# iden3/snarkjs

Measured on NVIDIA H100. Metric: groth16_proofs_per_sec, higher is better.
Workload: dtype u32x8 (256-bit modular integers, 32-bit limbs)

## Files before the change

### snarkjs_b200/csrc/ec.cuh

```cuda
#pragma once
#include "fp.cuh"

namespace sb {

template <class P> struct Fp2 {
    typedef Fp<P> B;
    static constexpr bool HAS_MUL2 = false;
    B a, b;
    SB_HD static Fp2 one() { Fp2 r; r.a = B::one(); r.b = B::zero(); return r; }
    SB_HD static Fp2 inv(const Fp2& x) {
        B t = B::inv_binary(B::add(B::sqr(x.a), B::sqr(x.b)));
        Fp2 r; r.a = B::mul(x.a, t); r.b = B::neg(B::mul(x.b, t)); return r;
    }
    SB_HD static Fp2 zero() { Fp2 r; r.a = B::zero(); r.b = B::zero(); return r; }
    SB_HD bool is_zero() const { return a.is_zero() & b.is_zero(); }
    SB_HD bool operator==(const Fp2& o) const { return (a == o.a) & (b == o.b); }
    SB_HD static Fp2 add(const Fp2& x, const Fp2& y) { Fp2 r; r.a = B::add(x.a, y.a); r.b = B::add(x.b, y.b); return r; }
    SB_HD static Fp2 sub(const Fp2& x, const Fp2& y) { Fp2 r; r.a = B::sub(x.a, y.a); r.b = B::sub(x.b, y.b); return r; }
    SB_HD static Fp2 dbl(const Fp2& x) { Fp2 r; r.a = B::dbl(x.a); r.b = B::dbl(x.b); return r; }
    SB_HD static Fp2 neg(const Fp2& x) { Fp2 r; r.a = B::neg(x.a); r.b = B::neg(x.b); return r; }
    SB_HD static Fp2 cneg(const Fp2& x, bool f) { Fp2 r; r.a = B::cneg(x.a, f); r.b = B::cneg(x.b, f); return r; }
    SB_HD_NOINLINE static Fp2 mul(const Fp2& x, const Fp2& y) { return mul_i(x, y); }
    SB_HD_NOINLINE static Fp2 sqr(const Fp2& x) { return sqr_i(x); }
    SB_HD static Fp2 mul_i(const Fp2& x, const Fp2& y) {
#if defined(__CUDA_ARCH__) && defined(SB_FP2_LAZY)
        return mul_lazy(x, y);
#endif
        if constexpr (B::HAS_MUL2) {
            Fp2 r; r.a = B::mul2(x.a, y.a, x.b, B::neg(y.b)); r.b = B::mul2(x.a, y.b, x.b, y.a); return r;
        } else {
            B A = B::mul(x.a, y.a), Bb = B::mul(x.b, y.b);
            B C = B::mul(B::add(x.a, x.b), B::add(y.a, y.b));
            Fp2 r; r.a = B::sub(A, Bb); r.b = B::sub(B::sub(C, A), Bb); return r;
        }
    }
    SB_HD static Fp2 mul_lazy(const Fp2& x, const Fp2& y) {
        constexpr int N = B::N;
        uint32_t v0[2 * N], v1[2 * N], v2[2 * N], sa[N], sb[N];
        B::mul_wide(x.a.v, y.a.v, v0);
        B::mul_wide(x.b.v, y.b.v, v1);
        B::add_noreduce(x.a, x.b, sa); B::add_noreduce(y.a, y.b, sb);
        B::mul_wide(sa, sb, v2);
        B::wide_sub(v2, v0); B::wide_sub(v2, v1);
        uint32_t bw = B::wide_sub(v0, v1);
        B::wide_add_p_high(v0, bw);
        Fp2 r; r.a = B::redc_wide(v0); r.b = B::redc_wide(v2); return r;
    }
    SB_HD static Fp2 sqr_i(const Fp2& x) {
        B AB = B::mul(x.a, x.b);
        Fp2 r; r.a = B::mul(B::add(x.a, x.b), B::sub(x.a, x.b)); r.b = B::dbl(AB); return r;
    }
};

template <class F> struct Affine {
    F x, y;
    SB_HD bool is_inf() const { return x.is_zero() & y.is_zero(); }
};

template <class F> struct XYZZ {
    F x, y, zz, zzz;
    SB_HD static XYZZ inf() { XYZZ r; r.x = F::zero(); r.y = F::zero(); r.zz = F::zero(); r.zzz = F::zero(); return r; }
    SB_HD bool is_inf() const { return zz.is_zero(); }

    SB_HD_NOINLINE static XYZZ dbl_affine(const F& px, const F& py, const F& one) {
        XYZZ r;
        if (py.is_zero()) return inf();
        F U = F::dbl(py), V = F::sqr(U), W = F::mul(U, V), S = F::mul(px, V);
        F M = F::sqr(px); M = F::add(F::dbl(M), M);
        r.x = F::sub(F::sqr(M), F::dbl(S));
        r.y = F::sub(F::mul(M, F::sub(S, r.x)), F::mul(W, py));
        r.zz = V; r.zzz = W;
        (void)one;
        return r;
    }
    SB_HD_NOINLINE static XYZZ dbl(const XYZZ& p) {
        if (p.is_inf() || p.y.is_zero()) return inf();
        XYZZ r;
        F U = F::dbl(p.y), V = F::sqr(U), W = F::mul(U, V), S = F::mul(p.x, V);
        F M = F::sqr(p.x); M = F::add(F::dbl(M), M);
        r.x = F::sub(F::sqr(M), F::dbl(S));
        r.y = F::sub(F::mul(M, F::sub(S, r.x)), F::mul(W, p.y));
        r.zz = F::mul(V, p.zz); r.zzz = F::mul(W, p.zzz);
        return r;
    }
    SB_HD void add_affine(const F& qx, const F& qy, const F& one) {
        if (is_inf()) { x = qx; y = qy; zz = one; zzz = one; return; }
        F U2 = F::mul_i(qx, zz), S2 = F::mul_i(qy, zzz);
        F Pp = F::sub(U2, x), R = F::sub(S2, y);
        if (Pp.is_zero()) {
            if (R.is_zero()) *this = dbl_affine(qx, qy, one);
            else *this = inf();
            return;
        }
        F PP = F::sqr_i(Pp), PPP = F::mul_i(Pp, PP), Q = F::mul_i(x, PP);
        F X3 = F::sub(F::sub(F::sqr_i(R), PPP), F::dbl(Q));
        F Y3;
        if constexpr (F::HAS_MUL2) Y3 = F::mul2_i(R, F::sub(Q, X3), F::neg(y), PPP);
        else Y3 = F::sub(F::mul_i(R, F::sub(Q, X3)), F::mul_i(y, PPP));
        x = X3; y = Y3; zz = F::mul_i(zz, PP); zzz = F::mul_i(zzz, PPP);
    }
    SB_HD void add_i(const XYZZ& q) {
        if (q.is_inf()) return;
        if (is_inf()) { *this = q; return; }
        F U1 = F::mul_i(x, q.zz), S1 = F::mul_i(y, q.zzz);
        F ZZ = F::mul_i(zz, q.zz), ZZZ = F::mul_i(zzz, q.zzz);
        F Pp = F::sub(F::mul_i(q.x, zz), U1), R = F::sub(F::mul_i(q.y, zzz), S1);
        if (Pp.is_zero()) {
            if (R.is_zero()) *this = dbl(*this);
            else *this = inf();
            return;
        }
        F PP = F::sqr_i(Pp), PPP = F::mul_i(Pp, PP), Q = F::mul_i(U1, PP);
        F X3 = F::sub(F::sub(F::sqr_i(R), PPP), F::dbl(Q));
        F Y3;
        if constexpr (F::HAS_MUL2) Y3 = F::mul2_i(R, F::sub(Q, X3), F::neg(S1), PPP);
        else Y3 = F::sub(F::mul_i(R, F::sub(Q, X3)), F::mul_i(S1, PPP));
        x = X3; y = Y3; zz = F::mul_i(ZZ, PP); zzz = F::mul_i(ZZZ, PPP);
    }
    SB_HD void add(const XYZZ& q) {
        if (q.is_inf()) return;
        if (is_inf()) { *this = q; return; }
        F U1 = F::mul(x, q.zz), U2 = F::mul(q.x, zz);
        F S1 = F::mul(y, q.zzz), S2 = F::mul(q.y, zzz);
        F Pp = F::sub(U2, U1), R = F::sub(S2, S1);
        if (Pp.is_zero()) {
            if (R.is_zero()) *this = dbl(*this);
            else *this = inf();
            return;
        }
        F PP = F::sqr(Pp), PPP = F::mul(Pp, PP), Q = F::mul(U1, PP);
        F X3 = F::sub(F::sub(F::sqr(R), PPP), F::dbl(Q));
        F Y3 = F::sub(F::mul(R, F::sub(Q, X3)), F::mul(S1, PPP));
        x = X3; y = Y3;
        zz = F::mul(F::mul(zz, q.zz), PP); zzz = F::mul(F::mul(zzz, q.zzz), PPP);
    }
};

}
```

### snarkjs_b200/csrc/fp.cuh

```cuda
#pragma once
#include <cstdint>

namespace sb {

#ifdef __CUDACC__
#define SB_CONSTEXPR_HD __host__ __device__
#else
#define SB_CONSTEXPR_HD
#endif
#define SB_L(...) {__VA_ARGS__}
#define SB_FIELD_TAG(NAME, NLIMBS, NP0, PL, ONEL, R2L)                                          \
    struct NAME {                                                                             \
        static constexpr int N = NLIMBS;                                                      \
        static constexpr uint32_t np0 = NP0;                                                  \
        SB_CONSTEXPR_HD static constexpr uint32_t p(int i)   { constexpr uint32_t v[NLIMBS] = PL;   return v[i]; } \
        SB_CONSTEXPR_HD static constexpr uint32_t one(int i) { constexpr uint32_t v[NLIMBS] = ONEL; return v[i]; } \
        SB_CONSTEXPR_HD static constexpr uint32_t r2(int i)  { constexpr uint32_t v[NLIMBS] = R2L;  return v[i]; } \
    };

SB_FIELD_TAG(BnFq, 8, 0xe4866389u,
    SB_L(0xd87cfd47u, 0x3c208c16u, 0x6871ca8du, 0x97816a91u, 0x8181585du, 0xb85045b6u, 0xe131a029u, 0x30644e72u),
    SB_L(0xc58f0d9du, 0xd35d438du, 0xf5c70b3du, 0x0a78eb28u, 0x7879462cu, 0x666ea36fu, 0x9a07df2fu, 0x0e0a77c1u),
    SB_L(0x538afa89u, 0xf32cfc5bu, 0xd44501fbu, 0xb5e71911u, 0x0a417ff6u, 0x47ab1effu, 0xcab8351fu, 0x06d89f71u))
SB_FIELD_TAG(BnFr, 8, 0xefffffffu,
    SB_L(0xf0000001u, 0x43e1f593u, 0x79b97091u, 0x2833e848u, 0x8181585du, 0xb85045b6u, 0xe131a029u, 0x30644e72u),
    SB_L(0x4ffffffbu, 0xac96341cu, 0x9f60cd29u, 0x36fc7695u, 0x7879462eu, 0x666ea36fu, 0x9a07df2fu, 0x0e0a77c1u),
    SB_L(0xae216da7u, 0x1bb8e645u, 0xe35c59e3u, 0x53fe3ab1u, 0x53bb8085u, 0x8c49833du, 0x7f4e44a5u, 0x0216d0b1u))
SB_FIELD_TAG(BlsFq, 12, 0xfffcfffdu,
    SB_L(0xffffaaabu, 0xb9feffffu, 0xb153ffffu, 0x1eabfffeu, 0xf6b0f624u, 0x6730d2a0u, 0xf38512bfu, 0x64774b84u, 0x434bacd7u, 0x4b1ba7b6u, 0x397fe69au, 0x1a0111eau),
    SB_L(0x0002fffdu, 0x76090000u, 0xc40c0002u, 0xebf4000bu, 0x53c758bau, 0x5f489857u, 0x70525745u, 0x77ce5853u, 0xa256ec6du, 0x5c071a97u, 0xfa80e493u, 0x15f65ec3u),
    SB_L(0x1c341746u, 0xf4df1f34u, 0x09d104f1u, 0x0a76e6a6u, 0x4c95b6d5u, 0x8de5476cu, 0x939d83c0u, 0x67eb88a9u, 0xb519952du, 0x9a793e85u, 0x92cae3aau, 0x11988fe5u))
SB_FIELD_TAG(BlsFr, 8, 0xffffffffu,
    SB_L(0x00000001u, 0xffffffffu, 0xfffe5bfeu, 0x53bda402u, 0x09a1d805u, 0x3339d808u, 0x299d7d48u, 0x73eda753u),
    SB_L(0xfffffffeu, 0x00000001u, 0x00034802u, 0x5884b7fau, 0xecbc4ff5u, 0x998c4fefu, 0xacc5056fu, 0x1824b159u),
    SB_L(0xf3f29c6du, 0xc999e990u, 0x87925c23u, 0x2b6cedcbu, 0x7254398fu, 0x05d31496u, 0x9f59ff11u, 0x0748d9d9u))

#ifdef __CUDACC__
#define SB_HD __host__ __device__ __forceinline__
#define SB_HD_NOINLINE __host__ __device__ __noinline__
#else
#define SB_HD inline
#define SB_HD_NOINLINE inline
#endif

namespace ptx {
#ifdef __CUDA_ARCH__
#define SB_ASM(...) asm volatile(__VA_ARGS__)
SB_HD uint32_t mul_lo(uint32_t a, uint32_t b) { uint32_t r; SB_ASM("mul.lo.u32 %0, %1, %2;" : "=r"(r) : "r"(a), "r"(b)); return r; }
SB_HD uint32_t mul_hi(uint32_t a, uint32_t b) { uint32_t r; SB_ASM("mul.hi.u32 %0, %1, %2;" : "=r"(r) : "r"(a), "r"(b)); return r; }
SB_HD void mad_lo_cc(uint32_t& acc, uint32_t a, uint32_t b)  { SB_ASM("mad.lo.cc.u32 %0, %1, %2, %0;"  : "+r"(acc) : "r"(a), "r"(b)); }
SB_HD void madc_lo_cc(uint32_t& acc, uint32_t a, uint32_t b) { SB_ASM("madc.lo.cc.u32 %0, %1, %2, %0;" : "+r"(acc) : "r"(a), "r"(b)); }
SB_HD void madc_hi_cc(uint32_t& acc, uint32_t a, uint32_t b) { SB_ASM("madc.hi.cc.u32 %0, %1, %2, %0;" : "+r"(acc) : "r"(a), "r"(b)); }
SB_HD void madc_lo_cc3(uint32_t& r, uint32_t a, uint32_t b, uint32_t c) { SB_ASM("madc.lo.cc.u32 %0, %1, %2, %3;" : "=r"(r) : "r"(a), "r"(b), "r"(c)); }
SB_HD void madc_hi_cc3(uint32_t& r, uint32_t a, uint32_t b, uint32_t c) { SB_ASM("madc.hi.cc.u32 %0, %1, %2, %3;" : "=r"(r) : "r"(a), "r"(b), "r"(c)); }
SB_HD void madc_hi3(uint32_t& r, uint32_t a, uint32_t b, uint32_t c)    { SB_ASM("madc.hi.u32 %0, %1, %2, %3;"    : "=r"(r) : "r"(a), "r"(b), "r"(c)); }
SB_HD void add_cc(uint32_t& r, uint32_t a, uint32_t b)  { SB_ASM("add.cc.u32 %0, %1, %2;"  : "=r"(r) : "r"(a), "r"(b)); }
SB_HD void addc_cc(uint32_t& r, uint32_t a, uint32_t b) { SB_ASM("addc.cc.u32 %0, %1, %2;" : "=r"(r) : "r"(a), "r"(b)); }
SB_HD void addc(uint32_t& r, uint32_t a, uint32_t b)    { SB_ASM("addc.u32 %0, %1, %2;"    : "=r"(r) : "r"(a), "r"(b)); }
SB_HD void sub_cc(uint32_t& r, uint32_t a, uint32_t b)  { SB_ASM("sub.cc.u32 %0, %1, %2;"  : "=r"(r) : "r"(a), "r"(b)); }
SB_HD void subc_cc(uint32_t& r, uint32_t a, uint32_t b) { SB_ASM("subc.cc.u32 %0, %1, %2;" : "=r"(r) : "r"(a), "r"(b)); }
SB_HD void subc(uint32_t& r, uint32_t a, uint32_t b)    { SB_ASM("subc.u32 %0, %1, %2;"    : "=r"(r) : "r"(a), "r"(b)); }
#else
static thread_local uint32_t g_cc = 0;
inline uint32_t mul_lo(uint32_t a, uint32_t b) { return (uint32_t)((uint64_t)a * b); }
inline uint32_t mul_hi(uint32_t a, uint32_t b) { return (uint32_t)(((uint64_t)a * b) >> 32); }
inline uint32_t emu_add(uint32_t a, uint32_t b, uint32_t cin, bool setcc) { uint64_t t = (uint64_t)a + b + cin; if (setcc) g_cc = (uint32_t)(t >> 32); return (uint32_t)t; }
inline uint32_t emu_sub(uint32_t a, uint32_t b, uint32_t bin, bool setcc) { uint64_t t = (uint64_t)a - b - bin; if (setcc) g_cc = (uint32_t)((t >> 32) & 1); return (uint32_t)t; }
inline void mad_lo_cc(uint32_t& acc, uint32_t a, uint32_t b)  { acc = emu_add(mul_lo(a, b), acc, 0, true); }
inline void madc_lo_cc(uint32_t& acc, uint32_t a, uint32_t b) { acc = emu_add(mul_lo(a, b), acc, g_cc, true); }
inline void madc_hi_cc(uint32_t& acc, uint32_t a, uint32_t b) { acc = emu_add(mul_hi(a, b), acc, g_cc, true); }
inline void madc_lo_cc3(uint32_t& r, uint32_t a, uint32_t b, uint32_t c) { r = emu_add(mul_lo(a, b), c, g_cc, true); }
inline void madc_hi_cc3(uint32_t& r, uint32_t a, uint32_t b, uint32_t c) { r = emu_add(mul_hi(a, b), c, g_cc, true); }
inline void madc_hi3(uint32_t& r, uint32_t a, uint32_t b, uint32_t c)    { r = emu_add(mul_hi(a, b), c, g_cc, false); }
inline void add_cc(uint32_t& r, uint32_t a, uint32_t b)  { r = emu_add(a, b, 0, true); }
inline void addc_cc(uint32_t& r, uint32_t a, uint32_t b) { r = emu_add(a, b, g_cc, true); }
inline void addc(uint32_t& r, uint32_t a, uint32_t b)    { r = emu_add(a, b, g_cc, false); }
inline void sub_cc(uint32_t& r, uint32_t a, uint32_t b)  { r = emu_sub(a, b, 0, true); }
inline void subc_cc(uint32_t& r, uint32_t a, uint32_t b) { r = emu_sub(a, b, g_cc, true); }
inline void subc(uint32_t& r, uint32_t a, uint32_t b)    { r = emu_sub(a, b, g_cc, false); }
#endif
}

template <class P> struct Fp {
    static constexpr int N = P::N;
    static constexpr bool HAS_MUL2 = P::p(P::N - 1) < 0x55555555u;
    uint32_t v[N];

    SB_HD static Fp zero() { Fp r;
_Pragma("unroll")
        for (int i = 0; i < N; i++) r.v[i] = 0;
        return r; }
    SB_HD static Fp one() { Fp r;
_Pragma("unroll")
        for (int i = 0; i < N; i++) r.v[i] = P::one(i);
        return r; }
    SB_HD static Fp r2() { Fp r;
_Pragma("unroll")
        for (int i = 0; i < N; i++) r.v[i] = P::r2(i);
        return r; }
    SB_HD bool is_zero() const { uint32_t o = 0;
_Pragma("unroll")
        for (int i = 0; i < N; i++) o |= v[i];
        return o == 0; }
    SB_HD bool operator==(const Fp& b) const { uint32_t o = 0;
_Pragma("unroll")
        for (int i = 0; i < N; i++) o |= v[i] ^ b.v[i];
        return o == 0; }

    SB_HD static void final_sub(uint32_t* x) {
        uint32_t d[N], bw;
        ptx::sub_cc(d[0], x[0], P::p(0));
_Pragma("unroll")
        for (int i = 1; i < N; i++) ptx::subc_cc(d[i], x[i], P::p(i));
        ptx::subc(bw, 0, 0);
_Pragma("unroll")
        for (int i = 0; i < N; i++) x[i] = bw ? x[i] : d[i];
    }

    SB_HD static Fp add(const Fp& a, const Fp& b) {
        Fp r;
        ptx::add_cc(r.v[0], a.v[0], b.v[0]);
_Pragma("unroll")
        for (int i = 1; i < N - 1; i++) ptx::addc_cc(r.v[i], a.v[i], b.v[i]);
        ptx::addc(r.v[N - 1], a.v[N - 1], b.v[N - 1]);
        final_sub(r.v);
        return r;
    }
    SB_HD static Fp dbl(const Fp& a) { return add(a, a); }
    SB_HD static Fp sub(const Fp& a, const Fp& b) {
        Fp r; uint32_t bw;
        ptx::sub_cc(r.v[0], a.v[0], b.v[0]);
_Pragma("unroll")
        for (int i = 1; i < N; i++) ptx::subc_cc(r.v[i], a.v[i], b.v[i]);
        ptx::subc(bw, 0, 0);
        ptx::add_cc(r.v[0], r.v[0], bw & P::p(0));
_Pragma("unroll")
        for (int i = 1; i < N - 1; i++) ptx::addc_cc(r.v[i], r.v[i], bw & P::p(i));
        ptx::addc(r.v[N - 1], r.v[N - 1], bw & P::p(N - 1));
        return r;
    }
    SB_HD static Fp neg(const Fp& a) {
        Fp r; uint32_t nz = a.is_zero() ? 0u : 0xffffffffu;
        ptx::sub_cc(r.v[0], nz & P::p(0), a.v[0]);
_Pragma("unroll")
        for (int i = 1; i < N - 1; i++) ptx::subc_cc(r.v[i], nz & P::p(i), a.v[i]);
        ptx::subc(r.v[N - 1], nz & P::p(N - 1), a.v[N - 1]);
        return r;
    }
    SB_HD static Fp cneg(const Fp& a, bool flag) {
        Fp n = neg(a), r;
_Pragma("unroll")
        for (int i = 0; i < N; i++) r.v[i] = flag ? n.v[i] : a.v[i];
        return r;
    }

    SB_HD static void row(uint32_t* X, uint32_t* Y, const uint32_t* a, uint32_t bi) {
        ptx::add_cc(Y[0], Y[0], X[1]);
_Pragma("unroll")
        for (int j = 0; j < N - 2; j += 2) {
            ptx::madc_lo_cc3(X[j], a[j + 1], bi, X[j + 2]);
            ptx::madc_hi_cc3(X[j + 1], a[j + 1], bi, X[j + 3]);
        }
        ptx::madc_lo_cc3(X[N - 2], a[N - 1], bi, 0);
        ptx::madc_hi3(X[N - 1], a[N - 1], bi, 0);
        ptx::mad_lo_cc(Y[0], a[0], bi);
        ptx::madc_hi_cc(Y[1], a[0], bi);
_Pragma("unroll")
        for (int j = 2; j < N; j += 2) {
            ptx::madc_lo_cc(Y[j], a[j], bi);
            ptx::madc_hi_cc(Y[j + 1], a[j], bi);
        }
        ptx::addc(X[N - 1], X[N - 1], 0);
        reduce(X, Y);
    }
    SB_HD static void reduce(uint32_t* X, uint32_t* Y) {
        uint32_t m = Y[0] * P::np0;
        ptx::mad_lo_cc(X[0], P::p(1), m);
        ptx::madc_hi_cc(X[1], P::p(1), m);
_Pragma("unroll")
        for (int j = 2; j < N; j += 2) {
            ptx::madc_lo_cc(X[j], P::p(j + 1), m);
            ptx::madc_hi_cc(X[j + 1], P::p(j + 1), m);
        }
        ptx::mad_lo_cc(Y[0], P::p(0), m);
        ptx::madc_hi_cc(Y[1], P::p(0), m);
_Pragma("unroll")
        for (int j = 2; j < N; j += 2) {
            ptx::madc_lo_cc(Y[j], P::p(j), m);
            ptx::madc_hi_cc(Y[j + 1], P::p(j), m);
        }
        ptx::addc(X[N - 1], X[N - 1], 0);
    }

    SB_HD static Fp mul(const Fp& a, const Fp& b) {
#if !defined(__CUDA_ARCH__) && !defined(SB_HOST_EMULATE_PTX)
        return host_mul(a, b);
#else
        uint32_t E[N], O[N];
_Pragma("unroll")
        for (int j = 0; j < N; j += 2) {
            E[j] = ptx::mul_lo(a.v[j], b.v[0]);     E[j + 1] = ptx::mul_hi(a.v[j], b.v[0]);
            O[j] = ptx::mul_lo(a.v[j + 1], b.v[0]); O[j + 1] = ptx::mul_hi(a.v[j + 1], b.v[0]);
        }
        reduce(O, E);
_Pragma("unroll")
        for (int i = 1; i < N; i += 2) {
            row(E, O, a.v, b.v[i]);
            if (i + 1 < N) row(O, E, a.v, b.v[i + 1]);
        }
        Fp r;
        ptx::add_cc(r.v[0], E[0], O[1]);
_Pragma("unroll")
        for (int i = 1; i < N - 1; i++) ptx::addc_cc(r.v[i], E[i], O[i + 1]);
        ptx::addc(r.v[N - 1], E[N - 1], 0);
        final_sub(r.v);
        return r;
#endif
    }
    SB_HD static Fp sqr(const Fp& a) { return mul(a, a); }

    SB_HD static void row2(uint32_t* X, uint32_t* Y, const uint32_t* a, uint32_t bi, const uint32_t* u, uint32_t vi) {
        ptx::add_cc(Y[0], Y[0], X[1]);
_Pragma("unroll")
        for (int j = 0; j < N - 2; j += 2) {
            ptx::madc_lo_cc3(X[j], a[j + 1], bi, X[j + 2]);
            ptx::madc_hi_cc3(X[j + 1], a[j + 1], bi, X[j + 3]);
        }
        ptx::madc_lo_cc3(X[N - 2], a[N - 1], bi, 0);
        ptx::madc_hi3(X[N - 1], a[N - 1], bi, 0);
        ptx::mad_lo_cc(Y[0], a[0], bi);
        ptx::madc_hi_cc(Y[1], a[0], bi);
_Pragma("unroll")
        for (int j = 2; j < N; j += 2) {
            ptx::madc_lo_cc(Y[j], a[j], bi);
            ptx::madc_hi_cc(Y[j + 1], a[j], bi);
        }
        ptx::addc(X[N - 1], X[N - 1], 0);
        add_product(X, Y, u, vi);
        reduce(X, Y);
    }
    SB_HD static void add_product(uint32_t* X, uint32_t* Y, const uint32_t* u, uint32_t vi) {
        ptx::mad_lo_cc(X[0], u[1], vi);
        ptx::madc_hi_cc(X[1], u[1], vi);
_Pragma("unroll")
        for (int j = 2; j < N; j += 2) {
            ptx::madc_lo_cc(X[j], u[j + 1], vi);
            ptx::madc_hi_cc(X[j + 1], u[j + 1], vi);
        }
        ptx::mad_lo_cc(Y[0], u[0], vi);
        ptx::madc_hi_cc(Y[1], u[0], vi);
_Pragma("unroll")
        for (int j = 2; j < N; j += 2) {
            ptx::madc_lo_cc(Y[j], u[j], vi);
            ptx::madc_hi_cc(Y[j + 1], u[j], vi);
        }
        ptx::addc(X[N - 1], X[N - 1], 0);
    }
    SB_HD static Fp mul2(const Fp& x, const Fp& y, const Fp& u, const Fp& v) {
        static_assert(P::p(N - 1) < 0x55555555u, "mul2 needs 3p < R");
#if !defined(__CUDA_ARCH__) && !defined(SB_HOST_EMULATE_PTX)
        return add(host_mul(x, y), host_mul(u, v));
#else
        uint32_t E[N], O[N];
_Pragma("unroll")
        for (int j = 0; j < N; j += 2) {
            E[j] = ptx::mul_lo(x.v[j], y.v[0]);     E[j + 1] = ptx::mul_hi(x.v[j], y.v[0]);
            O[j] = ptx::mul_lo(x.v[j + 1], y.v[0]); O[j + 1] = ptx::mul_hi(x.v[j + 1], y.v[0]);
        }
        add_product(O, E, u.v, v.v[0]);
        reduce(O, E);
_Pragma("unroll")
        for (int i = 1; i < N; i += 2) {
            row2(E, O, x.v, y.v[i], u.v, v.v[i]);
            if (i + 1 < N) row2(O, E, x.v, y.v[i + 1], u.v, v.v[i + 1]);
        }
        Fp r;
        ptx::add_cc(r.v[0], E[0], O[1]);
_Pragma("unroll")
        for (int i = 1; i < N - 1; i++) ptx::addc_cc(r.v[i], E[i], O[i + 1]);
        ptx::addc(r.v[N - 1], E[N - 1], 0);
        final_sub(r.v);
        return r;
#endif
    }
    SB_HD static void mul_wide(const uint32_t* a, const uint32_t* b, uint32_t* T) {
        uint32_t E[2 * N], O[2 * N];
_Pragma("unroll")
        for (int k = 0; k < 2 * N; k++) { E[k] = 0; O[k] = 0; }
_Pragma("unroll")
        for (int i = 0; i < N; i++) {
            const uint32_t bi = b[i];
            if ((i & 1) == 0) {
                ptx::mad_lo_cc(E[i], a[0], bi); ptx::madc_hi_cc(E[i + 1], a[0], bi);
_Pragma("unroll")
                for (int j = 2; j < N; j += 2) { ptx::madc_lo_cc(E[i + j], a[j], bi); ptx::madc_hi_cc(E[i + j + 1], a[j], bi); }
                ptx::addc(E[i + N], E[i + N], 0);
                ptx::mad_lo_cc(O[i], a[1], bi); ptx::madc_hi_cc(O[i + 1], a[1], bi);
_Pragma("unroll")
                for (int j = 3; j < N; j += 2) { ptx::madc_lo_cc(O[i + j - 1], a[j], bi); ptx::madc_hi_cc(O[i + j], a[j], bi); }
                ptx::addc(O[i + N], O[i + N], 0);
            } else {
                ptx::mad_lo_cc(E[i + 1], a[1], bi); ptx::madc_hi_cc(E[i + 2], a[1], bi);
_Pragma("unroll")
                for (int j = 3; j < N; j += 2) { ptx::madc_lo_cc(E[i + j], a[j], bi); ptx::madc_hi_cc(E[i + j + 1], a[j], bi); }
                if (i + N + 1 < 2 * N) ptx::addc(E[i + N + 1], E[i + N + 1], 0);
                ptx::mad_lo_cc(O[i - 1], a[0], bi); ptx::madc_hi_cc(O[i], a[0], bi);
_Pragma("unroll")
                for (int j = 2; j < N; j += 2) { ptx::madc_lo_cc(O[i + j - 1], a[j], bi); ptx::madc_hi_cc(O[i + j], a[j], bi); }
                ptx::addc(O[i + N - 1], O[i + N - 1], 0);
            }
        }
        T[0] = E[0];
        ptx::add_cc(T[1], E[1], O[0]);
_Pragma("unroll")
        for (int k = 2; k < 2 * N - 1; k++) ptx::addc_cc(T[k], E[k], O[k - 1]);
        ptx::addc(T[2 * N - 1], E[2 * N - 1], O[2 * N - 2]);
    }
    SB_HD static void shift_in(uint32_t* X, uint32_t* Y, uint32_t t) {
        ptx::add_cc(Y[0], Y[0], X[1]);
_Pragma("unroll")
        for (int j = 0; j < N - 2; j++) ptx::addc_cc(X[j], X[j + 2], 0);
        ptx::addc_cc(X[N - 2], t, 0);
        ptx::addc(X[N - 1], 0, 0);
    }
    SB_HD static Fp redc_wide(const uint32_t* T) {
        uint32_t E[N], O[N];
_Pragma("unroll")
        for (int k = 0; k < N; k++) { E[k] = T[k]; O[k] = 0; }
        reduce(O, E);
_Pragma("unroll")
        for (int i = 1; i < N; i += 2) {
            shift_in(E, O, T[N + i - 1]); reduce(E, O);
            if (i + 1 < N) { shift_in(O, E, T[N + i]); reduce(O, E); }
        }
        Fp r;
        ptx::add_cc(r.v[0], E[0], O[1]);
_Pragma("unroll")
        for (int i = 1; i < N - 1; i++) ptx::addc_cc(r.v[i], E[i], O[i + 1]);
        ptx::addc(r.v[N - 1], E[N - 1], T[2 * N - 1]);
        final_sub(r.v);
        return r;
    }
    SB_HD static uint32_t wide_sub(uint32_t* x, const uint32_t* y) {
        uint32_t bw;
        ptx::sub_cc(x[0], x[0], y[0]);
_Pragma("unroll")
        for (int k = 1; k < 2 * N; k++) ptx::subc_cc(x[k], x[k], y[k]);
        ptx::subc(bw, 0, 0);
        return bw;
    }
    SB_HD static void wide_add_p_high(uint32_t* x, uint32_t mask) {
        ptx::add_cc(x[N], x[N], mask & P::p(0));
_Pragma("unroll")
        for (int k = 1; k < N - 1; k++) ptx::addc_cc(x[N + k], x[N + k], mask & P::p(k));
        ptx::addc(x[2 * N - 1], x[2 * N - 1], mask & P::p(N - 1));
    }
    SB_HD static void add_noreduce(const Fp& a, const Fp& b, uint32_t* out) {
        ptx::add_cc(out[0], a.v[0], b.v[0]);
_Pragma("unroll")
        for (int k = 1; k < N - 1; k++) ptx::addc_cc(out[k], a.v[k], b.v[k]);
        ptx::addc(out[N - 1], a.v[N - 1], b.v[N - 1]);
    }

    SB_HD static Fp mul2_i(const Fp& x, const Fp& y, const Fp& u, const Fp& v) {
        if constexpr (P::p(N - 1) < 0x55555555u) return mul2(x, y, u, v);
        else return add(mul(x, y), mul(u, v));
    }
    SB_HD static Fp mul_i(const Fp& a, const Fp& b) { return mul(a, b); }
    SB_HD static Fp sqr_i(const Fp& a) { return mul(a, a); }
    SB_HD static Fp to_mont(const Fp& a) { return mul(a, r2()); }

#ifndef __CUDA_ARCH__
    static inline Fp host_mul(const Fp& a, const Fp& b) {
        constexpr int M = N / 2;
        typedef unsigned __int128 u128;
        uint64_t A[M], B[M], Pm[M], t[M + 2];
        for (int i = 0; i < M; i++) {
            A[i] = a.v[2 * i] | ((uint64_t)a.v[2 * i + 1] << 32);
            B[i] = b.v[2 * i] | ((uint64_t)b.v[2 * i + 1] << 32);
            Pm[i] = P::p(2 * i) | ((uint64_t)P::p(2 * i + 1) << 32);
        }
        for (int i = 0; i < M + 2; i++) t[i] = 0;
        uint64_t inv = (uint32_t)(0u - P::np0);
        inv *= 2 - Pm[0] * inv;
        const uint64_t n0 = 0 - inv;
        for (int i = 0; i < M; i++) {
            u128 c = 0;
            for (int j = 0; j < M; j++) { c += (u128)A[j] * B[i] + t[j]; t[j] = (uint64_t)c; c >>= 64; }
            c += t[M]; t[M] = (uint64_t)c; t[M + 1] = (uint64_t)(c >> 64);
            const uint64_t m = t[0] * n0;
            c = ((u128)m * Pm[0] + t[0]) >> 64;
            for (int j = 1; j < M; j++) { c += (u128)m * Pm[j] + t[j]; t[j - 1] = (uint64_t)c; c >>= 64; }
            c += t[M]; t[M - 1] = (uint64_t)c; t[M] = t[M + 1] + (uint64_t)(c >> 64);
        }
        bool ge = t[M] != 0;
        if (!ge) { ge = true; for (int i = M - 1; i >= 0; i--) { if (t[i] > Pm[i]) break; if (t[i] < Pm[i]) { ge = false; break; } } }
        if (ge) { u128 bw = 0; for (int i = 0; i < M; i++) { u128 d = (u128)t[i] - Pm[i] - bw; t[i] = (uint64_t)d; bw = (d >> 64) & 1; } }
        Fp r;
        for (int i = 0; i < M; i++) { r.v[2 * i] = (uint32_t)t[i]; r.v[2 * i + 1] = (uint32_t)(t[i] >> 32); }
        return r;
    }
#endif
    SB_HD static Fp pow(const Fp& a, const uint32_t* e, int nw) {
        Fp r = one();
        for (int i = nw * 32 - 1; i >= 0; i--) {
            r = sqr(r);
            if ((e[i >> 5] >> (i & 31)) & 1) r = mul(r, a);
        }
        return r;
    }
    SB_HD static Fp inv_binary(const Fp& a) {
        if (a.is_zero()) return a;
        uint32_t u[N], v[N], r[N], s[N];
_Pragma("unroll")
        for (int i = 0; i < N; i++) { u[i] = P::p(i); v[i] = a.v[i]; r[i] = 0; s[i] = 0; }
        s[0] = 1;
        int k = 0;
        auto shr1 = [](uint32_t* x) {
_Pragma("unroll")
            for (int i = 0; i < N - 1; i++) x[i] = (x[i] >> 1) | (x[i + 1] << 31);
            x[N - 1] >>= 1; };
        auto shl1 = [](uint32_t* x) {
_Pragma("unroll")
            for (int i = N - 1; i > 0; i--) x[i] = (x[i] << 1) | (x[i - 1] >> 31);
            x[0] <<= 1; };
        auto sub = [](uint32_t* x, const uint32_t* y) { uint32_t bw = 0;
_Pragma("unroll")
            for (int i = 0; i < N; i++) { uint32_t xi = x[i], yi = y[i]; uint32_t d = xi - yi - bw; bw = (xi < yi) | ((xi == yi) & bw); x[i] = d; } };
        auto add = [](uint32_t* x, const uint32_t* y) { uint32_t c = 0;
_Pragma("unroll")
            for (int i = 0; i < N; i++) { uint32_t xi = x[i]; uint32_t t = xi + y[i]; uint32_t c1 = t < xi; uint32_t t2 = t + c; c = c1 | (t2 < t); x[i] = t2; } };
        auto gt = [](const uint32_t* x, const uint32_t* y) { bool g = false, decided = false;
_Pragma("unroll")
            for (int i = N - 1; i >= 0; i--) { bool ne = x[i] != y[i]; g = (!decided && ne) ? (x[i] > y[i]) : g; decided = decided || ne; }
            return g; };
        auto is0 = [](const uint32_t* x) { uint32_t o = 0;
_Pragma("unroll")
            for (int i = 0; i < N; i++) o |= x[i];
            return o == 0; };
        while (!is0(v)) {
            if (!(u[0] & 1)) { shr1(u); shl1(s); }
            else if (!(v[0] & 1)) { shr1(v); shl1(r); }
            else if (gt(u, v)) { sub(u, v); shr1(u); add(r, s); shl1(s); }
            else { sub(v, u); shr1(v); add(s, r); shl1(r); }
            k++;
        }
        uint32_t pp[N];
_Pragma("unroll")
        for (int i = 0; i < N; i++) pp[i] = P::p(i);
        if (!gt(pp, r)) sub(r, pp);
        sub(pp, r);
        Fp o;
_Pragma("unroll")
        for (int i = 0; i < N; i++) o.v[i] = pp[i];
        const int j = 64 * N - k;
        Fp t = one();
        for (int bit = 9; bit >= 0; bit--) { t = sqr(t); if ((j >> bit) & 1) t = dbl(t); }
        return mul(o, t);
    }
    SB_HD static Fp inv(const Fp& a) {
        uint32_t e[N];
        uint32_t bw = 2;
        for (int i = 0; i < N; i++) { uint32_t pi = P::p(i); e[i] = pi - bw; bw = pi < bw ? 1u : 0u; }
        return pow(a, e, N);
    }

    SB_HD static Fp from_mont(const Fp& a) { Fp o = zero(); o.v[0] = 1; return mul(a, o); }
};

}
```

Before: 34.99.

## Add dedicated Montgomery squaring and fused four-product mul4 for Fp2 mul2

Adds a squaring routine that skips redundant cross-product limbs by doubling the multiplicand, and routes sqr_i through it. Adds a mul4 that accumulates four products before each Montgomery reduction row, enabling Fp2::mul2_i (used in XYZZ Y3 computation) with a single reduction per output component. It also removes the SB_FP2_LAZY path. Together these aim to cut multiply and reduction instruction counts in the EC add inner loop of the MSM, at the cost of more register pressure and code size.

New measurement: 35.60 (median of 6 runs). 1.8% higher.

```diff
diff --git a/snarkjs_b200/csrc/ec.cuh b/snarkjs_b200/csrc/ec.cuh
--- a/snarkjs_b200/csrc/ec.cuh
+++ b/snarkjs_b200/csrc/ec.cuh
@@ -5,7 +5,6 @@
 
 template <class P> struct Fp2 {
     typedef Fp<P> B;
-    static constexpr bool HAS_MUL2 = false;
     B a, b;
     SB_HD static Fp2 one() { Fp2 r; r.a = B::one(); r.b = B::zero(); return r; }
     SB_HD static Fp2 inv(const Fp2& x) {
@@ -23,9 +22,6 @@
     SB_HD_NOINLINE static Fp2 mul(const Fp2& x, const Fp2& y) { return mul_i(x, y); }
     SB_HD_NOINLINE static Fp2 sqr(const Fp2& x) { return sqr_i(x); }
     SB_HD static Fp2 mul_i(const Fp2& x, const Fp2& y) {
-#if defined(__CUDA_ARCH__) && defined(SB_FP2_LAZY)
-        return mul_lazy(x, y);
-#endif
         if constexpr (B::HAS_MUL2) {
             Fp2 r; r.a = B::mul2(x.a, y.a, x.b, B::neg(y.b)); r.b = B::mul2(x.a, y.b, x.b, y.a); return r;
         } else {
@@ -33,6 +29,13 @@
             B C = B::mul(B::add(x.a, x.b), B::add(y.a, y.b));
             Fp2 r; r.a = B::sub(A, Bb); r.b = B::sub(B::sub(C, A), Bb); return r;
         }
+    }
+    static constexpr bool HAS_MUL2 = B::HAS_MUL4 && B::N <= 8;
+    SB_HD static Fp2 mul2_i(const Fp2& x, const Fp2& y, const Fp2& u, const Fp2& v) {
+        Fp2 r;
+        r.a = B::mul4(x.a, y.a, x.b, B::neg(y.b), u.a, v.a, u.b, B::neg(v.b));
+        r.b = B::mul4(x.a, y.b, x.b, y.a, u.a, v.b, u.b, v.a);
+        return r;
     }
     SB_HD static Fp2 mul_lazy(const Fp2& x, const Fp2& y) {
         constexpr int N = B::N;
diff --git a/snarkjs_b200/csrc/fp.cuh b/snarkjs_b200/csrc/fp.cuh
--- a/snarkjs_b200/csrc/fp.cuh
+++ b/snarkjs_b200/csrc/fp.cuh
@@ -155,6 +155,10 @@
     }
 
     SB_HD static void row(uint32_t* X, uint32_t* Y, const uint32_t* a, uint32_t bi) {
+        row_product(X, Y, a, bi);
+        reduce(X, Y);
+    }
+    SB_HD static void row_product(uint32_t* X, uint32_t* Y, const uint32_t* a, uint32_t bi) {
         ptx::add_cc(Y[0], Y[0], X[1]);
 _Pragma("unroll")
         for (int j = 0; j < N - 2; j += 2) {
@@ -171,7 +175,6 @@
             ptx::madc_hi_cc(Y[j + 1], a[j], bi);
         }
         ptx::addc(X[N - 1], X[N - 1], 0);
-        reduce(X, Y);
     }
     SB_HD static void reduce(uint32_t* X, uint32_t* Y) {
         uint32_t m = Y[0] * P::np0;
@@ -217,25 +220,67 @@
         return r;
 #endif
     }
-    SB_HD static Fp sqr(const Fp& a) { return mul(a, a); }
-
-    SB_HD static void row2(uint32_t* X, uint32_t* Y, const uint32_t* a, uint32_t bi, const uint32_t* u, uint32_t vi) {
+    SB_HD static Fp sqr(const Fp& a) {
+#if !defined(__CUDA_ARCH__) && !defined(SB_HOST_EMULATE_PTX)
+        return host_mul(a, a);
+#else
+        if constexpr (!HAS_MUL2) return mul(a, a);
+        else {
+            uint32_t d[N];
+            d[0] = a.v[0] << 1;
+_Pragma("unroll")
+            for (int j = 1; j < N; j++) d[j] = (a.v[j] << 1) | (a.v[j - 1] >> 31);
+            uint32_t E[N], O[N], e[N];
+            sqr_multiplicand(a.v, d, 0, e);
+_Pragma("unroll")
+            for (int j = 0; j < N; j += 2) {
+                E[j] = ptx::mul_lo(e[j], a.v[0]);     E[j + 1] = ptx::mul_hi(e[j], a.v[0]);
+                O[j] = ptx::mul_lo(e[j + 1], a.v[0]); O[j + 1] = ptx::mul_hi(e[j + 1], a.v[0]);
+            }
+            reduce(O, E);
+_Pragma("unroll")
+            for (int i = 1; i < N; i += 2) {
+                sqr_multiplicand(a.v, d, i, e); row_lead(E, O, e, a.v[i], i); reduce(E, O);
+                if (i + 1 < N) { sqr_multiplicand(a.v, d, i + 1, e); row_lead(O, E, e, a.v[i + 1], i + 1); reduce(O, E); }
+            }
+            Fp r;
+            ptx::add_cc(r.v[0], E[0], O[1]);
+_Pragma("unroll")
+            for (int k = 1; k < N - 1; k++) ptx::addc_cc(r.v[k], E[k], O[k + 1]);
+            ptx::addc(r.v[N - 1], E[N - 1], 0);
+            final_sub(r.v);
+            return r;
+        }
+#endif
+    }
+    SB_HD static void sqr_multiplicand(const uint32_t* a, const uint32_t* d, int i, uint32_t* e) {
+_Pragma("unroll")
+        for (int j = 0; j < N; j++) e[j] = j < i ? 0u : j == i ? a[i] : j == i + 1 ? a[j] << 1 : d[j];
+    }
+    SB_HD static void row_lead(uint32_t* X, uint32_t* Y, const uint32_t* a, uint32_t bi, int lead) {
         ptx::add_cc(Y[0], Y[0], X[1]);
 _Pragma("unroll")
         for (int j = 0; j < N - 2; j += 2) {
-            ptx::madc_lo_cc3(X[j], a[j + 1], bi, X[j + 2]);
-            ptx::madc_hi_cc3(X[j + 1], a[j + 1], bi, X[j + 3]);
+            if (j + 1 < lead) { ptx::addc_cc(X[j], X[j + 2], 0); ptx::addc_cc(X[j + 1], X[j + 3], 0); }
+            else { ptx::madc_lo_cc3(X[j], a[j + 1], bi, X[j + 2]); ptx::madc_hi_cc3(X[j + 1], a[j + 1], bi, X[j + 3]); }
         }
         ptx::madc_lo_cc3(X[N - 2], a[N - 1], bi, 0);
         ptx::madc_hi3(X[N - 1], a[N - 1], bi, 0);
-        ptx::mad_lo_cc(Y[0], a[0], bi);
-        ptx::madc_hi_cc(Y[1], a[0], bi);
-_Pragma("unroll")
-        for (int j = 2; j < N; j += 2) {
-            ptx::madc_lo_cc(Y[j], a[j], bi);
-            ptx::madc_hi_cc(Y[j + 1], a[j], bi);
-        }
-        ptx::addc(X[N - 1], X[N - 1], 0);
+        const int first = (lead + 1) & ~1;
+        if (first < N) {
+            ptx::mad_lo_cc(Y[first], a[first], bi);
+            ptx::madc_hi_cc(Y[first + 1], a[first], bi);
+_Pragma("unroll")
+            for (int j = first + 2; j < N; j += 2) {
+                ptx::madc_lo_cc(Y[j], a[j], bi);
+                ptx::madc_hi_cc(Y[j + 1], a[j], bi);
+            }
+            ptx::addc(X[N - 1], X[N - 1], 0);
+        }
+    }
+
+    SB_HD static void row2(uint32_t* X, uint32_t* Y, const uint32_t* a, uint32_t bi, const uint32_t* u, uint32_t vi) {
+        row_product(X, Y, a, bi);
         add_product(X, Y, u, vi);
         reduce(X, Y);
     }
@@ -283,6 +328,42 @@
         return r;
 #endif
     }
+    static constexpr bool HAS_MUL4 = P::p(P::N - 1) < 0x33333333u;
+    SB_HD static Fp mul4(const Fp& x0, const Fp& y0, const Fp& x1, const Fp& y1, const Fp& x2, const Fp& y2, const Fp& x3, const Fp& y3) {
+        static_assert(HAS_MUL4, "mul4 needs 5p < R");
+#if !defined(__CUDA_ARCH__) && !defined(SB_HOST_EMULATE_PTX)
+        return add(add(host_mul(x0, y0), host_mul(x1, y1)), add(host_mul(x2, y2), host_mul(x3, y3)));
+#else
+        uint32_t E[N], O[N];
+_Pragma("unroll")
+        for (int j = 0; j < N; j += 2) {
+            E[j] = ptx::mul_lo(x0.v[j], y0.v[0]);     E[j + 1] = ptx::mul_hi(x0.v[j], y0.v[0]);
+            O[j] = ptx::mul_lo(x0.v[j + 1], y0.v[0]); O[j + 1] = ptx::mul_hi(x0.v[j + 1], y0.v[0]);
+        }
+        add_product(O, E, x1.v, y1.v[0]);
+        add_product(O, E, x2.v, y2.v[0]);
+        add_product(O, E, x3.v, y3.v[0]);
+        reduce(O, E);
+_Pragma("unroll")
+        for (int i = 1; i < N; i += 2) {
+            row_product(E, O, x0.v, y0.v[i]);
+            add_product(E, O, x1.v, y1.v[i]); add_product(E, O, x2.v, y2.v[i]); add_product(E, O, x3.v, y3.v[i]);
+            reduce(E, O);
+            if (i + 1 < N) {
+                row_product(O, E, x0.v, y0.v[i + 1]);
+                add_product(O, E, x1.v, y1.v[i + 1]); add_product(O, E, x2.v, y2.v[i + 1]); add_product(O, E, x3.v, y3.v[i + 1]);
+                reduce(O, E);
+            }
+        }
+        Fp r;
+        ptx::add_cc(r.v[0], E[0], O[1]);
+_Pragma("unroll")
+        for (int i = 1; i < N - 1; i++) ptx::addc_cc(r.v[i], E[i], O[i + 1]);
+        ptx::addc(r.v[N - 1], E[N - 1], 0);
+        final_sub(r.v);
+        return r;
+#endif
+    }
     SB_HD static void mul_wide(const uint32_t* a, const uint32_t* b, uint32_t* T) {
         uint32_t E[2 * N], O[2 * N];
 _Pragma("unroll")
@@ -367,7 +448,7 @@
         else return add(mul(x, y), mul(u, v));
     }
     SB_HD static Fp mul_i(const Fp& a, const Fp& b) { return mul(a, b); }
-    SB_HD static Fp sqr_i(const Fp& a) { return mul(a, a); }
+    SB_HD static Fp sqr_i(const Fp& a) { return sqr(a); }
     SB_HD static Fp to_mont(const Fp& a) { return mul(a, r2()); }
 
 #ifndef __CUDA_ARCH__
```
